# ilovin/lstm_ctc_ocr

Measured on NVIDIA H100. Metric: text-line images/sec (fwd+CTC loss), higher is better.
Workload: dtype bf16

## Files before the change

lstm_ctc_ocr_b200/csrc/backward.cu:

```cuda
#include <cmath>
#include <cstring>

#include "backward_kernels.cuh"
#include "conv1_wgrad_tc.cuh"
#include "conv_swap.cuh"
#include "gemm_launch.h"
#include "kernels.cuh"
#include "lstm_bwd.cuh"
#include "model_internal.h"

extern "C" int crnn_model_set_training(crnn_model* m, int flag) {
  if (!m) return crnn_fail(CRNN_INVALID_VALUE, "set_training: null model");
  if (flag && m->cfg.compute_dtype >= 2) return crnn_fail(CRNN_UNSUPPORTED, "set_training: the f32-class paths (compute_dtype 2, 3) are forward + CTC only");
  if (flag && !m->wblock_bwd) {
    const size_t nB[9] = {512 * 4608, 256 * 4608, 256 * 2304, 128 * 2304, 64 * 1152, 1024 * 1024, 512 * 64, 512 * 2048, 512 * 1024};
    size_t tot = 1024;
    for (size_t v : nB) tot += align_up(v * 2);
    CUDA_TRY(cudaMalloc(&m->wblock_bwd, tot));
    uint8_t* p = reinterpret_cast<uint8_t*>(m->wblock_bwd);
    __nv_bfloat16** dst[9] = {&m->Bd_c42, &m->Bd_c41, &m->Bd_c32, &m->Bd_c31, &m->Bd_c2, &m->Bd_c5, &m->Bld, &m->Bxb, &m->Bhb};
    for (int i = 0; i < 9; ++i) { *dst[i] = reinterpret_cast<__nv_bfloat16*>(p); p += align_up(nB[i] * 2); }
    m->grad_sumsq = reinterpret_cast<double*>(p);
    CRNN_TRY(make_tmap_2d(&m->tD_c42, m->Bd_c42, 512, 4608, 4608, 256));
    CRNN_TRY(make_tmap_2d(&m->tD_c41, m->Bd_c41, 256, 4608, 4608, 256));
// ... 102 lines not shown
    if (!attr) {
      CUDA_TRY(cudaFuncSetAttribute(lstm_bwd::lstm_bwd_kernel, cudaFuncAttributeMaxDynamicSharedMemorySize, lstm_bwd::SMEM_BYTES));
      CUDA_TRY(cudaFuncSetAttribute(lstm_bwd::lstm_bwd_ks_kernel, cudaFuncAttributeMaxDynamicSharedMemorySize, lstm_bwd::ks::SMEM_BYTES));
      attr = true;
    }
    cudaLaunchConfig_t cfg;
    memset(&cfg, 0, sizeof(cfg));
    cfg.gridDim = dim3(lstm_bwd::CS * 2 * lp.tiles_per_dir);
    cfg.blockDim = dim3(m->bptt_ks ? lstm_bwd::ks::NUM_THREADS : lstm_bwd::NUM_THREADS);
    cfg.dynamicSmemBytes = m->bptt_ks ? lstm_bwd::ks::SMEM_BYTES : lstm_bwd::SMEM_BYTES;
    cfg.stream = st;
    cudaLaunchAttribute at[1];
    at[0].id = cudaLaunchAttributeClusterDimension;
    at[0].val.clusterDim.x = lstm_bwd::CS; at[0].val.clusterDim.y = 1; at[0].val.clusterDim.z = 1;
    cfg.attrs = at; cfg.numAttrs = 1;
    if (m->bptt_ks) CUDA_TRY(cudaLaunchKernelEx(&cfg, lstm_bwd::lstm_bwd_ks_kernel, m->tD_h256, lp, pl.bptt_x));
    else CUDA_TRY(cudaLaunchKernelEx(&cfg, lstm_bwd::lstm_bwd_kernel, pl.tG_dzstate, m->tD_h, lp));
  }
  BMARK();
  {
    const std::string fw = "logits/bidirectional_rnn/fw/lstm_cell", bw = "logits/bidirectional_rnn/bw/lstm_cell";
    const long long dW = m->find(bw + "/weights")->offset - m->find(fw + "/weights")->offset;
    const long long db = m->find(bw + "/biases")->offset - m->find(fw + "/biases")->offset;
    CRNN_TRY(launch_colsum_bf16(pl.dz_all, R, 2048, G(fw + "/biases"), 32, db, st));
    {
      gemm_tn::Params p = tn_plain(512, 2048, R, G(fw + "/weights"), 1024);
      p.num_n_tiles = 8; p.lstm_cols = 1; p.dir_stride = dW;
      CRNN_TRY((launch_gemm_tn<256, gemm_tn::TN_PLAIN, 4>(pl.tT_a5, pl.tT_dz, p, sms, st)));
    }
    {
      gemm_tn::Params p = tn_plain(256, 1024, R, G(fw + "/weights"), 1024);
      p.num_n_tiles = 4; p.lstm_cols = 1; p.out_row_offset = 512; p.a_row_shift = -1;
// ... 216 lines not shown
```

lstm_ctc_ocr_b200/csrc/lstm.cuh:

```cuda
#pragma once
#include <cuda.h>

#include "common.cuh"
#include "wgmma.cuh"

namespace lstm {

constexpr int NUM_THREADS = 384;
constexpr int BLOCK_M = 128;

struct Params {
  const __nv_bfloat16* xproj;
  __nv_bfloat16* h_state;
  __nv_bfloat16* lstm_out;
  const int* seq_len;
  int Nimg, Npad, H, T, tiles_per_dir;
  __nv_bfloat16* gates;
  float* csave;
  int swap_ls;
  long long* trace;
};

#define LSTM_TRACE_WG(wg, ev)                                                                           \
  do {                                                                                                  \
    if (p.trace != nullptr && lane == 0 && s >= 8 && s < 12 && (blockIdx.x == 0 || blockIdx.x == 5))    \
      p.trace[((((blockIdx.x ? 1 : 0) * 2 + (wg)) * 4 + (s - 8)) * 16) + (ev)] = clock64();             \
  } while (0)
#define LSTM_TRACE(ev) LSTM_TRACE_WG(0, ev)

__device__ __forceinline__ uint32_t cluster_ctarank() {
  uint32_t r;
  asm volatile("mov.u32 %0, %%cluster_ctarank;" : "=r"(r));
  return r;
}
__device__ __forceinline__ void cluster_arrive_release() { asm volatile("barrier.cluster.arrive.release.aligned;" ::: "memory"); }
// ... 197 lines not shown
  static constexpr int HALF_ROWS = BLOCK_M / 2;
  static constexpr int HALF_A_BYTES = 32 * HALF_ROWS * 16;
  static constexpr int A_BYTES = 2 * HALF_A_BYTES;
  static constexpr int SLICE_BYTES = HALF_A_BYTES / CS;
  static constexpr int BAR_OFFSET = 2 * A_BYTES + B_BYTES;
  static constexpr int SMEM_BYTES = BAR_OFFSET + 128 + 1024;
};

__device__ __forceinline__ void bulk_copy_s2s_cluster(uint32_t dst_cluster_addr, const void* src_smem, uint32_t bytes,
                                                      uint32_t bar_cluster_addr) {
  asm volatile("cp.async.bulk.shared::cluster.shared::cta.mbarrier::complete_tx::bytes [%0], [%1], %2, [%3];" ::"r"(dst_cluster_addr),
               "r"(ptx::smem_u32(src_smem)), "r"(bytes), "r"(bar_cluster_addr)
               : "memory");
}

template <int CS, int MODE, int EW>
__global__ void __launch_bounds__(McThreads<EW>::ALL, 1)
lstm_mc_kernel(const __grid_constant__ CUtensorMap tmW, const Params p) {
  static_assert(CS == 8, "8 CTAs x 32 units");
  using C = CfgMc<CS>;
  constexpr int UPC = C::UPC, NCOLS = C::NCOLS;
  static_assert(EW == 8, "epilogue warps = the two MMA warpgroups");
  static_assert(NCOLS == 128, "fragment column group j = gate j/4, units 8(j%4) ..: one m64n128 product per half and step");
  constexpr bool DS = (MODE == 1), MS = (MODE == 2), GX = (MODE == 3), LOCAL = DS || MS;
  constexpr uint32_t FILL_TX = LOCAL ? (CS - 1) * C::SLICE_BYTES : C::HALF_A_BYTES;

  extern __shared__ uint8_t smem_raw[];
  uint8_t* smem = smem_raw + ((1024u - (ptx::smem_u32(smem_raw) & 1023u)) & 1023u);
  uint8_t* smem_a = smem;
  uint8_t* smem_b = smem + 2 * C::A_BYTES;
  uint64_t* a_full = reinterpret_cast<uint64_t*>(smem + C::BAR_OFFSET);
  uint64_t* b_full = a_full + 4;
  uint64_t* part_ready = b_full + 1;

  const int warp_idx = threadIdx.x >> 5, lane = threadIdx.x & 31;
  const int rank = (int)cluster_ctarank();
  const int unit = blockIdx.x / CS;
  const int dir = unit / p.tiles_per_dir;
  const int tile = unit - dir * p.tiles_per_dir;

  if (warp_idx == 0 && lane == 0) {
    ptx::prefetch_tmap(&tmW);
    for (int i = 0; i < 4; ++i) {
      ptx::mbar_init(&part_ready[i], CS);
      ptx::mbar_init(&a_full[i], GX ? 128 : LOCAL ? 2 : 1);
    }
    ptx::mbar_init(b_full, 1);
    ptx::fence_barrier_init();
    for (int hf = 0; hf < 2; ++hf) {
      if (!GX && p.T > 1) ptx::mbar_arrive_expect_tx(&a_full[2 * hf + 1], FILL_TX);
      if (!GX && p.T > 2) ptx::mbar_arrive_expect_tx(&a_full[2 * hf + 0], FILL_TX);
    }
    ptx::mbar_arrive_expect_tx(b_full, C::B_BYTES);
    for (int kb = 0; kb < 4; ++kb)
      ptx::tma_load_2d(&tmW, b_full, smem_b + kb * NCOLS * 128, kb * 64, dir * 1024 + rank * NCOLS);
  }
  __syncthreads();
  cluster_arrive_release();
  cluster_wait_acquire();

  if (warp_idx < 4) {
    ptx::setmaxnreg_dec<40>();
  } else {
    ptx::setmaxnreg_inc<232>();
    const int wgi = (warp_idx >> 2) - 1;
    const int w = warp_idx & 3, q4 = lane & 3;
    const int rr0 = 16 * w + (lane >> 2);
    int n[2], len[2];
    bool okn[2];
#pragma unroll
    for (int rh = 0; rh < 2; ++rh) {
      n[rh] = tile * BLOCK_M + wgi * C::HALF_ROWS + rr0 + 8 * rh;
      okn[rh] = n[rh] < p.Nimg;
      len[rh] = okn[rh] ? min(max(__ldg(p.seq_len + n[rh]), 0), p.T) : 0;
    }
    float cst[2][4][2];
#pragma unroll
    for (int rh = 0; rh < 2; ++rh)
#pragma unroll
      for (int k = 0; k < 4; ++k) { cst[rh][k][0] = 0.f; cst[rh][k][1] = 0.f; }
    uint64_t* my_full = a_full + 2 * wgi;
    uint64_t* my_ready = part_ready + 2 * wgi;
    ptx::mbar_wait(b_full, 0);
    const uint32_t word_off = rr0 * 16 + q4 * 4;
    uint8_t* hx_half = reinterpret_cast<uint8_t*>(p.h_state) + (size_t)(unit * 2 + wgi) * C::HALF_A_BYTES;
    const size_t hx_buf_stride = (size_t)2 * p.tiles_per_dir * C::A_BYTES;

    for (int s = 0; s < p.T; ++s) {
      bool active[2];
      int t[2];
      uint32_t xw[2][4][4];
#pragma unroll
      for (int rh = 0; rh < 2; ++rh) {
        active[rh] = s < len[rh];
        t[rh] = active[rh] ? (dir ? (len[rh] - 1 - s) : s) : s;
        if (active[rh]) {
          const uint32_t* src = reinterpret_cast<const uint32_t*>(p.xproj + ((size_t)n[rh] * p.H + s) * 2048 + dir * 1024 + rank * NCOLS + 2 * q4);
#pragma unroll
          for (int g = 0; g < 4; ++g)
#pragma unroll
            for (int k = 0; k < 4; ++k) xw[rh][g][k] = __ldg(src + (g * UPC + 8 * k) / 2);
// ... 79 lines not shown
                ptx::mbar_arrive(&my_full[nb]);
              } else {
                const uint32_t dst_peer = ptx::mapa(ptx::smem_u32(my_slice), (uint32_t)lane);
                const uint32_t bar = ptx::mapa(ptx::smem_u32(&my_full[nb]), (uint32_t)lane);
                bulk_copy_s2s_cluster(dst_peer, my_slice, C::SLICE_BYTES, bar);
              }
            }
          } else if (MS) {
            if (lane == 0) {
              ptx::bulk_store_1d(hx_slice, my_slice, C::SLICE_BYTES);
              ptx::bulk_commit();
              asm volatile("cp.async.bulk.wait_group 0;" ::: "memory");
              ptx::bulk_load_1d_mc(my_slice, hx_slice, C::SLICE_BYTES, &my_full[nb], (uint16_t)(((1u << CS) - 1) & ~(1u << rank)));
              ptx::mbar_arrive(&my_full[nb]);
            }
          } else if (GX) {
            if (lane < CS) ptx::mbar_arrive_cluster(ptx::mapa(ptx::smem_u32(&my_ready[nb]), (uint32_t)lane));
          } else if (lane == 0) {
            ptx::bulk_load_1d_mc(my_slice, hx_slice, C::SLICE_BYTES, &my_full[nb], (uint16_t)((1u << CS) - 1));
          }
          __syncwarp();
          LSTM_TRACE_WG(wgi, 9);
        }
        if (GX) {
          ptx::mbar_wait_cluster(&my_ready[nb], (uint32_t)(s >> 1) & 1u);
          const uint8_t* g = hx_half + (size_t)nb * hx_buf_stride;
          uint8_t* a = smem_a + nb * C::A_BYTES + wgi * C::HALF_A_BYTES;
          const int et = threadIdx.x & 127;
          uint4 v[C::HALF_A_BYTES / 16 / 128];
#pragma unroll
// ... 20 lines not shown
          for (int g = 0; g < 4; ++g)
#pragma unroll
            for (int k = 0; k < 4; ++k)
              *reinterpret_cast<uint32_t*>(gs + g * LSTM_GATE_STRIDE + k * LSTM_GCHUNK_STRIDE) =
                  ptx::pack_bf16x2(d[16 * g + 4 * k + 2 * rh], d[16 * g + 4 * k + 2 * rh + 1]);
#pragma unroll
          for (int k = 0; k < 4; ++k)
            *reinterpret_cast<float2*>(cs + (2 * k + (q4 >> 1)) * LSTM_CCHUNK_STRIDE) = make_float2(cst[rh][k][0], cst[rh][k][1]);
        }
      }
      if (w == 0) LSTM_TRACE_WG(wgi, 10);
    }
  }

  __syncthreads();
  cluster_arrive_release();
  cluster_wait_acquire();
}

}
```

lstm_ctc_ocr_b200/csrc/lstm_bwd.cuh:

```cuda
#pragma once
#include <cuda.h>

#include "common.cuh"
#include "lstm.cuh"
#include "wgmma.cuh"

namespace lstm_bwd {

constexpr int NUM_THREADS = 256;
constexpr int BLOCK_M = 128;
constexpr int CS = 8;
constexpr int UPC = 32;
constexpr int STAGES = 6;
constexpr int B_BYTES = 16 * UPC * 128;
constexpr int A_STAGE = BLOCK_M * 128;
constexpr int ACC_OFFSET = B_BYTES + STAGES * A_STAGE;
constexpr int BAR_OFFSET = ACC_OFFSET + BLOCK_M * UPC * 4;
constexpr int SMEM_BYTES = BAR_OFFSET + 256 + 1024;

struct Params {
  const __nv_bfloat16* gates;
  const float* csave;
  const __nv_bfloat16* d_out;
  __nv_bfloat16* dz_state;
  __nv_bfloat16* dz_all;
  const int* seq_len;
  int Nimg, Npad, H, T, tiles_per_dir;
};

__device__ __forceinline__ uint4 pack8(const float* v) {
  return make_uint4(ptx::pack_bf16x2(v[0], v[1]), ptx::pack_bf16x2(v[2], v[3]), ptx::pack_bf16x2(v[4], v[5]),
                    ptx::pack_bf16x2(v[6], v[7]));
}
__device__ __forceinline__ void unpack8(const uint4 q, float* v) {
  v[0] = ptx::bf16_lo(q.x); v[1] = ptx::bf16_hi(q.x); v[2] = ptx::bf16_lo(q.y); v[3] = ptx::bf16_hi(q.y);
  v[4] = ptx::bf16_lo(q.z); v[5] = ptx::bf16_hi(q.z); v[6] = ptx::bf16_lo(q.w); v[7] = ptx::bf16_hi(q.w);
}

__global__ void __launch_bounds__(NUM_THREADS, 1)
lstm_bwd_kernel(const __grid_constant__ CUtensorMap tmDz, const __grid_constant__ CUtensorMap tmW, const Params p) {
  extern __shared__ uint8_t smem_raw[];
  uint8_t* smem = reinterpret_cast<uint8_t*>((reinterpret_cast<uintptr_t>(smem_raw) + 1023) & ~uintptr_t(1023));
// ... 183 lines not shown
  extern __shared__ uint8_t smem_raw[];
  uint8_t* smem = smem_raw + ((1024u - (ptx::smem_u32(smem_raw) & 1023u)) & 1023u);
  uint8_t* smem_b = smem;
  uint8_t* smem_a = smem + ks::B_BYTES;
  float* acc_tile = reinterpret_cast<float*>(smem + ks::ACC_OFFSET);
  uint64_t* b_full = reinterpret_cast<uint64_t*>(smem + ks::BAR_OFFSET);
  uint64_t* a_ready = b_full + 1;
  uint64_t* part_ready = a_ready + 1;

  const int warp_idx = threadIdx.x >> 5, lane = threadIdx.x & 31;
  const int rank = (int)lstm::cluster_ctarank();
  const int unit = blockIdx.x / CS;
  const int dir = unit / p.tiles_per_dir;
  const int tile = unit - dir * p.tiles_per_dir;
  const int num_units = 2 * p.tiles_per_dir;

  if (warp_idx == 0 && lane == 0) {
    ptx::prefetch_tmap(&tmW);
    ptx::mbar_init(b_full, 1);
    ptx::mbar_init(a_ready, ks::EPI_THREADS);
    ptx::mbar_init(&part_ready[0], CS);
    ptx::mbar_init(&part_ready[1], CS);
    ptx::fence_barrier_init();
    ptx::mbar_arrive_expect_tx(b_full, ks::B_BYTES);
    for (int kb = 0; kb < 2; ++kb) ptx::tma_load_2d(&tmW, b_full, smem_b + kb * 256 * 128, rank * 128 + kb * 64, dir * 256);
  }
  __syncthreads();
  lstm::cluster_arrive_release();
  lstm::cluster_wait_acquire();

// ... 140 lines not shown
        ptx::mbar_arrive(a_ready);
      }
      if (okn) {
        __nv_bfloat16* za = p.dz_all + ((size_t)n * p.H + t) * 2048 + dir * 1024 + rank * 128 + u0;
        ptx::st_global_v8(za + 0 * 32, zi0.x, zi0.y, zi0.z, zi0.w, zi1.x, zi1.y, zi1.z, zi1.w);
        ptx::st_global_v8(za + 1 * 32, zj0.x, zj0.y, zj0.z, zj0.w, zj1.x, zj1.y, zj1.z, zj1.w);
        ptx::st_global_v8(za + 2 * 32, zf0.x, zf0.y, zf0.z, zf0.w, zf1.x, zf1.y, zf1.z, zf1.w);
        ptx::st_global_v8(za + 3 * 32, zo0.x, zo0.y, zo0.z, zo0.w, zo1.x, zo1.y, zo1.z, zo1.w);
      }
    }
  }

  __syncthreads();
  lstm::cluster_arrive_release();
  lstm::cluster_wait_acquire();
}

}
```

lstm_ctc_ocr_b200/csrc/model.cu:

```cuda
#include <cstdarg>
#include <cstring>
#include <string>
#include <vector>

#include <cstdlib>
#include <condition_variable>
#include <mutex>
#include <thread>

#include "gemm_launch.h"
#include "lstm.cuh"
#include "conv_swap.cuh"
#include "conv1_tc.cuh"
#include "kernels.cuh"
#include "model_internal.h"

static thread_local char g_err[1024] = "";
int crnn_fail(int status, const char* fmt, ...) {
  va_list ap;
  va_start(ap, fmt);
  vsnprintf(g_err, sizeof(g_err), fmt, ap);
  va_end(ap);
  return status;
}
// ... 147 lines not shown
  if (prop.major != 9) {
    delete m;
    return crnn_fail(CRNN_UNSUPPORTED, "model_create: needs sm_90 (found sm_%d%d)", prop.major, prop.minor);
  }
  m->num_sms = prop.multiProcessorCount;
  if (const char* e = getenv("CRNN_BPTT")) m->bptt_ks = std::string(e) != "ring";
  if (const char* e = getenv("CRNN_CONV1")) m->conv1_tc = std::string(e) != "simt";
  if (const char* e = getenv("CRNN_BN_FUSE")) m->bn_red_fused = std::string(e) != "0";
  if (const char* e = getenv("CRNN_RELU_FUSE")) m->relu_mask_fused = std::string(e) != "0";
  if (const char* e = getenv("CRNN_CONV1_WGRAD")) m->conv1_wgrad_tc = std::string(e) != "simt";
  if (const char* e = getenv("CRNN_CONV2_DGRAD")) m->conv2_dgrad_swap = std::string(e) != "old";
  if (const char* e = getenv("CRNN_CONV2_WGRAD")) m->conv2_wgrad_swap = std::string(e) != "old";
  if (const char* e = getenv("CRNN_CONV2")) m->conv2_swap = std::string(e) != "pos";
  if (const char* e = getenv("CRNN_LSTM_IMPL")) {
    m->lstm_upc = (std::string(e) == "step") ? 64 : 32;
    m->lstm_mc = std::string(e) == "ds" ? 2 : std::string(e) == "mc" ? 1 : std::string(e) == "gx" ? 4 : (std::string(e) == "persistent" || std::string(e) == "step") ? 0 : 3;
  }

  const size_t nB[9] = {128 * 576, 256 * 1152, 256 * 2304, 512 * 2304, 512 * 4608, 512 * 2048, 2048 * 512, 2048 * 256, 64 * 512};
  size_t tot = 0;
  for (size_t v : nB) tot += (v * 2 + 1023) / 1024 * 1024;
  tot += 2048 * 4 + 1024;
  if (cudaMalloc(&m->wblock, tot) != cudaSuccess) { delete m; return crnn_fail(CRNN_CUDA_ERROR, "model_create: cudaMalloc"); }
  uint8_t* p = reinterpret_cast<uint8_t*>(m->wblock);
  __nv_bfloat16** dst[9] = {&m->Bc2, &m->Bc31, &m->Bc32, &m->Bc41, &m->Bc42, &m->Bc5, &m->Bx, &m->Bh, &m->Bl};
  for (int i = 0; i < 9; ++i) { *dst[i] = reinterpret_cast<__nv_bfloat16*>(p); p += (nB[i] * 2 + 1023) / 1024 * 1024; }
  m->xbias = reinterpret_cast<float*>(p); p += 2048 * 4;
  m->sumsq = reinterpret_cast<double*>(p);
  int st = CRNN_OK;
  if (st == CRNN_OK) st = make_tmap_2d(&m->tB_c2, m->Bc2, 128, 576, 576, 128);
  if (st == CRNN_OK) st = make_tmap_2d(&m->tB_c31, m->Bc31, 256, 1152, 1152, 256);
// ... 4 lines not shown
  if (st == CRNN_OK) st = make_tmap_2d(&m->tB_x, m->Bx, 2048, 512, 512, 256);
  if (st == CRNN_OK) st = make_tmap_2d(&m->tB_h, m->Bh, 2048, 256, 256, 256);
  if (st == CRNN_OK) st = make_tmap_2d(&m->tB_h128, m->Bh, 2048, 256, 256, 128);
  if (st == CRNN_OK) st = make_tmap_2d(&m->tB_l, m->Bl, 64, 512, 512, 64);
  if (st != CRNN_OK) { cudaFree(m->wblock); delete m; return st; }
  *out = m;
  return CRNN_OK;
}

extern "C" int crnn_model_destroy(crnn_model* m) {
  if (!m) return CRNN_OK;
  x3_destroy(m);
  if (m->wblock) cudaFree(m->wblock);
  if (m->wblock_bwd) cudaFree(m->wblock_bwd);
  if (m->d_peers) cudaFree(m->d_peers);
  for (auto e : m->prof_events) cudaEventDestroy(e);
  for (auto e : m->prof_events_bwd) cudaEventDestroy(e);
  for (auto e : m->chunk_events) cudaEventDestroy(e);
  delete m;
  return CRNN_OK;
}
extern "C" int crnn_num_tensors(const crnn_model* m) { return m ? (int)m->tensors.size() : 0; }
extern "C" int64_t crnn_param_count(const crnn_model* m) { return m ? m->total : 0; }
extern "C" int crnn_param_info(const crnn_model* m, int index, const char** tf_name, int64_t* offset, int64_t shape[4],
                               int* ndim) {
  if (!m || index < 0 || index >= (int)m->tensors.size()) return crnn_fail(CRNN_INVALID_VALUE, "param_info: bad index");
  const TensorInfo& t = m->tensors[index];
  if (tf_name) *tf_name = t.name.c_str();
  if (offset) *offset = t.offset;
  if (shape) for (int k = 0; k < 4; ++k) shape[k] = t.shape[k];
// ... 27 lines not shown
    CRNN_TRY(launch_transpose_cast(w, 512, 1024, 1024, m->Bx + (size_t)d * 1024 * 512, 512, m->lstm_upc, st));
    CRNN_TRY(launch_transpose_cast(w + 512 * 1024, 256, 1024, 1024, m->Bh + (size_t)d * 1024 * 256, 256, m->lstm_upc, st));
  }
  CRNN_TRY(launch_lstm_bias_prep(m->P(std::string(dirs[0]) + "/biases"), m->P(std::string(dirs[1]) + "/biases"), m->xbias, m->lstm_upc, st));
  CRNN_TRY(launch_transpose_cast(m->P("logits/weights"), 512, 64, 64, m->Bl, 512, 0, st));
  SumsqSegs segs;
  segs.n = 0;
  for (auto& c : kConvs) {
    const TensorInfo* t = m->find(std::string(c.name) + "/weights");
    segs.off[segs.n] = t->offset; segs.cnt[segs.n] = t->count; segs.n++;
  }
  const TensorInfo* t = m->find("logits/weights");
  segs.off[segs.n] = t->offset; segs.cnt[segs.n] = t->count; segs.n++;
  CRNN_TRY(launch_sumsq(m->params, segs, m->sumsq, st));
  m->dirty = false;
  return CRNN_OK;
}

size_t align_up(size_t v, size_t a) { return (v + a - 1) / a * a; }

size_t layout_plan(Plan& pl, int N, int W, uint8_t* base, bool train) {
  pl.N = N; pl.W = W; pl.H1 = W / 2; pl.H2 = W / 4; pl.T = W / 4 - 1;
  pl.Npad = (N + 127) / 128 * 128;
  size_t off = 0;
  auto take = [&](size_t bytes) { uint8_t* p = base ? base + off : nullptr; off += align_up(bytes); return p; };
  const size_t n = N, h1 = pl.H1, h2 = pl.H2;
  pl.a1 = (__nv_bfloat16*)take(n * h1 * 16 * 64 * 2);
  pl.a2 = (__nv_bfloat16*)take(n * h2 * 8 * 128 * 2);
  pl.a3 = (__nv_bfloat16*)take(n * h2 * 8 * 256 * 2);
  pl.a3p = (__nv_bfloat16*)take(n * h2 * 4 * 256 * 2);
  pl.a4a_pre = (__nv_bfloat16*)take(n * h2 * 4 * 512 * 2);
  pl.a4a = (__nv_bfloat16*)take(n * h2 * 4 * 512 * 2);
  pl.a4b_pre = (__nv_bfloat16*)take(n * h2 * 4 * 512 * 2);
  pl.a4b = (__nv_bfloat16*)take(n * h2 * 2 * 512 * 2);
  pl.a5 = (__nv_bfloat16*)take(n * h2 * 512 * 2);
  pl.xproj = (__nv_bfloat16*)take(n * h2 * 2048 * 2);
  pl.lstm_out = (__nv_bfloat16*)take(n * h2 * 512 * 2);
  pl.h_state = (__nv_bfloat16*)take((size_t)2 * 2 * pl.Npad * 256 * 2);
  pl.c_state = (float*)take((size_t)2 * pl.Npad * 256 * 4);
  pl.stats = (double*)take(2 * 2 * 512 * 8);
  pl.bn = (float*)take(2 * 4 * 512 * 4);
  pl.train = train;
  if (train) {
    const size_t T = pl.T;
    pl.am1 = (uint8_t*)take(n * h1 * 16 * 64);
    pl.am2 = (uint8_t*)take(n * h2 * 8 * 128);
    pl.am3 = (uint8_t*)take(n * h2 * 4 * 256);
    pl.gates = (__nv_bfloat16*)take((size_t)2 * pl.Npad * T * 1024 * 2);
    pl.csave = (float*)take((size_t)2 * pl.Npad * T * 256 * 4);
    pl.dl_rows = (__nv_bfloat16*)take(n * h2 * 64 * 2);
    pl.d_lstm_out = (__nv_bfloat16*)take(n * h2 * 512 * 2);
    pl.dz_all = (__nv_bfloat16*)take(n * h2 * 2048 * 2);
    pl.dz_state = (__nv_bfloat16*)take((size_t)2 * 2 * pl.Npad * 1024 * 2);
// ... 315 lines not shown
    else CRNN_TRY((launch_gemm<256, gemm::A_PLAIN, gemm::EPI_BIAS_BF16, 4>(pl.tA_x, m->tB_x, p, sms, st, &pl.tO_x)));
  }
  STAGE_MARK();
  if (m->lstm_upc == 32) {
    constexpr int CS = 8;
    lstm::Params lp;
    lp.xproj = pl.xproj; lp.h_state = pl.h_state; lp.lstm_out = pl.lstm_out; lp.seq_len = time_step_len;
    lp.Nimg = N; lp.Npad = pl.Npad; lp.H = H2; lp.T = T; lp.tiles_per_dir = pl.Npad / 128;
    lp.gates = pl.train ? pl.gates : nullptr; lp.csave = pl.train ? pl.csave : nullptr;
    static long long* d_trace = nullptr;
    const bool want_trace = getenv("CRNN_LSTM_TRACE") != nullptr;
    if (want_trace && d_trace == nullptr) CUDA_TRY(cudaMalloc(&d_trace, 2 * 2 * 4 * 16 * sizeof(long long)));
    if (want_trace) CUDA_TRY(cudaMemsetAsync(d_trace, 0, 2 * 2 * 4 * 16 * sizeof(long long), st));
    lp.trace = want_trace ? d_trace : nullptr;
    lp.swap_ls = getenv("CRNN_LSTM_SWAPLS") != nullptr;
    auto kern = lstm::lstm_persistent_kernel<CS>;
    auto kern_mc = lstm::lstm_mc_kernel<CS, 0, 8>;
    auto kern_ds = lstm::lstm_mc_kernel<CS, 1, 8>;
    auto kern_ms = lstm::lstm_mc_kernel<CS, 2, 8>;
    auto kern_gx = lstm::lstm_mc_kernel<CS, 3, 8>;
    static bool attr = false;
    if (!attr) {
      CUDA_TRY(cudaFuncSetAttribute(kern, cudaFuncAttributeMaxDynamicSharedMemorySize, lstm::Cfg<CS>::SMEM_BYTES));
      CUDA_TRY(cudaFuncSetAttribute(kern_mc, cudaFuncAttributeMaxDynamicSharedMemorySize, lstm::CfgMc<CS>::SMEM_BYTES));
      CUDA_TRY(cudaFuncSetAttribute(kern_ds, cudaFuncAttributeMaxDynamicSharedMemorySize, lstm::CfgMc<CS>::SMEM_BYTES));
      CUDA_TRY(cudaFuncSetAttribute(kern_ms, cudaFuncAttributeMaxDynamicSharedMemorySize, lstm::CfgMc<CS>::SMEM_BYTES));
      CUDA_TRY(cudaFuncSetAttribute(kern_gx, cudaFuncAttributeMaxDynamicSharedMemorySize, lstm::CfgMc<CS>::SMEM_BYTES));
      attr = true;
    }
    cudaLaunchConfig_t cfg;
    memset(&cfg, 0, sizeof(cfg));
    cfg.gridDim = dim3(CS * 2 * lp.tiles_per_dir);
    cfg.blockDim = dim3(m->lstm_mc ? lstm::McThreads<8>::ALL : lstm::NUM_THREADS);
    cfg.dynamicSmemBytes = m->lstm_mc ? lstm::CfgMc<CS>::SMEM_BYTES : lstm::Cfg<CS>::SMEM_BYTES;
    cfg.stream = st;
    cudaLaunchAttribute at[1];
    at[0].id = cudaLaunchAttributeClusterDimension;
    at[0].val.clusterDim.x = CS; at[0].val.clusterDim.y = 1; at[0].val.clusterDim.z = 1;
    cfg.attrs = at; cfg.numAttrs = 1;
    if (m->lstm_mc == 4) CUDA_TRY(cudaLaunchKernelEx(&cfg, kern_gx, m->tB_h128, lp));
    else if (m->lstm_mc == 3) CUDA_TRY(cudaLaunchKernelEx(&cfg, kern_ms, m->tB_h128, lp));
    else if (m->lstm_mc == 2) CUDA_TRY(cudaLaunchKernelEx(&cfg, kern_ds, m->tB_h128, lp));
    else if (m->lstm_mc == 1) CUDA_TRY(cudaLaunchKernelEx(&cfg, kern_mc, m->tB_h128, lp));
    else CUDA_TRY(cudaLaunchKernelEx(&cfg, kern, pl.tA_hall, m->tB_h128, lp));
    if (want_trace) {
      long long h[2 * 2 * 4 * 16];
      CUDA_TRY(cudaStreamSynchronize(st));
      CUDA_TRY(cudaMemcpy(h, d_trace, sizeof(h), cudaMemcpyDeviceToHost));
      for (int c = 0; c < 2; ++c) {
        long long t0 = 0;
        for (int i = c * 128; i < (c + 1) * 128; ++i)
          if (h[i] && (!t0 || h[i] < t0)) t0 = h[i];
        for (int wg = 0; wg < 2; ++wg)
          for (int s = 0; s < 4; ++s) {
            const long long* r = h + ((c * 2 + wg) * 4 + s) * 16;
            bool any = false;
            for (int e = 0; e < 16; ++e) any = any || r[e];
            if (!any) continue;
            fprintf(stderr, "lstm_trace cta%d wg%d step%d:", c ? 5 : 0, wg, 8 + s);
// ... 196 lines not shown
```

lstm_ctc_ocr_b200/csrc/model_internal.h:

```cpp
#pragma once
#include <string>
#include <vector>

#include <cuda.h>

#include "common.cuh"
#include "gemm.cuh"

int make_tmap_2d(CUtensorMap* m, const void* base, uint64_t rows, uint64_t cols, uint64_t row_stride, uint32_t box_rows);
int make_tmap_nhwc(CUtensorMap* m, const void* base, int N, int H, int Wd, int C, int bh);
int make_tmap_2d_f32(CUtensorMap* m, const void* base, uint64_t rows, uint64_t cols, uint64_t row_stride, uint32_t box_rows);
int make_tmap_nhwc_f32(CUtensorMap* m, const void* base, int N, int H, int Wd, int C, int bh);
size_t align_up(size_t v, size_t a = 1024);
int make_tmap_2d_box(CUtensorMap* m, const void* base, uint64_t rows, uint64_t cols, uint64_t row_stride, uint32_t box_cols,
                     uint32_t box_rows);

struct TensorInfo {
  std::string name;
  int ndim;
  int64_t shape[4];
  int64_t offset;
  int64_t count;
};

// ... 6 lines not shown
static const char* kStageNames[] = {"conv1_pool1", "conv2_pool2", "conv3_1", "conv3_2_pool", "conv4_1_gemm", "bn4_1_apply",
                                    "conv4_2_gemm", "bn4_2_apply_pool3", "conv5", "lstm_xproj", "lstm_recurrence", "logits"};
static const int kNumStages = 12;
static const char* kBwdStageNames[] = {"zero+logits_bwd", "lstm_bptt", "lstm_wgrad+dx", "conv5_bwd", "bn4_2_bwd", "conv4_2_wgrad",
                                       "conv4_2_dgrad", "bn4_1_bwd", "conv4_1_wgrad", "conv4_1_dgrad", "conv3_2_bwd_elem", "conv3_2_wgrad",
                                       "conv3_2_dgrad", "conv3_1_bwd_elem", "conv3_1_wgrad", "conv3_1_dgrad", "conv2_bwd_elem", "conv2_wgrad",
                                       "conv2_dgrad", "conv1_wgrad"};
static const int kNumBwdStages = 20;

static const int kMaxChunks = 16;

struct Plan {
  int N = 0, W = 0, H1 = 0, H2 = 0, T = 0, Npad = 0;
  void* ws = nullptr;
  __nv_bfloat16 *a1, *a2, *a3, *a3p, *a4a_pre, *a4a, *a4b_pre, *a4b, *a5, *xproj, *lstm_out, *h_state;
  float* c_state;
  double* stats;
  float* bn;
  CUtensorMap tA_c2s;
  CUtensorMap tA_c2, tA_c31, tA_c32, tA_c41, tA_c42, tA_c5, tA_x, tA_h[2], tA_l, tA_hall;
  CUtensorMap tO_c1, tO_c2s, tO_c32, tO_c41, tO_c42, tO_x;
  int mg2 = 0, mg3 = 0, mg4 = 0, wm2 = 0, wm3 = 0, wm4 = 0;
  CUtensorMap tW_a1, tW_a2, tW_a3, tW_a3p, tW_a4a, tW_p4b, tW_p4a, tW_p32, tW_p31, tW_p2;
  bool train = false;
  uint8_t *am1, *am2, *am3;
  __nv_bfloat16* gates;
  float* csave;
  __nv_bfloat16 *dl_rows, *d_lstm_out, *dz_all, *dz_state, *d_a5, *d_a4b, *d_pre4b, *d_pre4a, *d_a3p, *d_pre32, *d_pre31, *d_a2,
      *d_pre2, *d_a1;
  uint8_t* bptt_x;
// ... 21 lines not shown
  bool dirty_bwd = true;
  void* wblock_bwd = nullptr;
  __nv_bfloat16 *Bd_c42 = nullptr, *Bd_c41, *Bd_c32, *Bd_c31, *Bd_c2, *Bd_c5, *Bld, *Bxb, *Bhb;
  CUtensorMap tD_c42, tD_c41, tD_c32, tD_c31, tD_c2, tD_c5, tD_l, tD_x, tD_h;
  CUtensorMap tDs_c2;
  CUtensorMap tD_h256;
  bool bptt_ks = true;
  double* grad_sumsq = nullptr;
  bool conv1_tc = true;
  bool bn_red_fused = true;
  bool relu_mask_fused = true;
  bool conv1_wgrad_tc = true;
  bool conv2_dgrad_swap = true;
  bool conv2_wgrad_swap = true;
  bool conv2_swap = true;
  int lstm_mc = 3;
  int lstm_upc = 32;
  Plan plan;
  void* x3 = nullptr;
  int dp_rank = 0, dp_world = 1;
  crnn_allreduce_fn xchg_cb = nullptr;
  void* xchg_user = nullptr;
  void** d_peers = nullptr;
  int* d_peer_err = nullptr;
  unsigned long long peer_epoch = 0;
  int bwd_sm_reserve = 0;
  crnn_grad_ready_fn grad_cb = nullptr;
  void* grad_user = nullptr;
  std::vector<cudaEvent_t> chunk_events;
  std::vector<cudaEvent_t> prof_events;
  int prof_slots = 0, prof_used = 0;
// ... 8 lines not shown
  float* P(const std::string& n) const { return params + find(n)->offset; }
};

size_t x3_workspace_size(int N, int W);
int x3_forward(crnn_model* m, const float* data, const int* time_step_len, int N, int W, float* logits_out, void* workspace,
               size_t workspace_bytes, cudaStream_t st);
int x3_debug_tap(crnn_model* m, const char* name, float* dst, size_t dst_elems, void* workspace, cudaStream_t st);
int x3_debug_tap_raw(crnn_model* m, const char* name, void* dst, size_t dst_bytes, void* workspace, cudaStream_t st);
void x3_destroy(crnn_model* m);
void x3_params_changed(crnn_model* m);

int dp_allreduce_1024(crnn_model* m, const double* in, double* out, cudaStream_t st);
int dp_allreduce_bn_finalize(crnn_model* m, double* stats, double count_global, const float* gamma, const float* beta, float eps,
                             float* bn , cudaStream_t st);

size_t layout_plan(Plan& pl, int N, int W, uint8_t* base, bool train);
int prepare_weights(crnn_model* m, cudaStream_t st);
int ensure_plan(crnn_model* m, int N, int W, void* ws, cudaStream_t st);

static inline gemm::Params conv_params(int N, int H, int Wd, int Cin, int Cout, int block_n, const float* bias, void* out,
                                       int merged = 0) {
  gemm::Params p;
  memset(&p, 0, sizeof(p));
  p.bh = 32 / Wd;
  p.Wd = Wd; p.H = H; p.Nimg = N;
  p.sb_per_img = (H + p.bh - 1) / p.bh;
  p.num_m_tiles = (N * p.sb_per_img + 3) / 4;
  p.num_n_tiles = Cout / block_n;
  p.cin_blocks = Cin / 64;
  p.num_k_blocks = 9 * p.cin_blocks;
// ... 9 lines not shown
```

lstm_ctc_ocr_b200/csrc/ptx.cuh:

```cuda
#pragma once
#include <cuda_runtime.h>
#include <cuda_bf16.h>
#include <stdint.h>

namespace ptx {

__device__ __forceinline__ uint32_t smem_u32(const void* p) {
  return static_cast<uint32_t>(__cvta_generic_to_shared(p));
}
__device__ __forceinline__ uint32_t lane_id() { return threadIdx.x & 31; }

__device__ __forceinline__ bool elect_one() {
  uint32_t pred = 0;
  asm volatile(
      "{\n\t.reg .pred p;\n\t"
      "elect.sync _|p, 0xffffffff;\n\t"
      "selp.u32 %0, 1, 0, p;\n\t}\n"
      : "=r"(pred));
  return pred != 0;
}

__device__ __forceinline__ void mbar_init(uint64_t* bar, uint32_t count) {
  asm volatile("mbarrier.init.shared::cta.b64 [%0], %1;" ::"r"(smem_u32(bar)), "r"(count));
}
// ... 163 lines not shown
__device__ __forceinline__ void mbar_wait_cluster(uint64_t* bar, uint32_t parity) {
  uint32_t ok;
  do {
    asm volatile(
        "{\n\t.reg .pred p;\n\t"
        "mbarrier.try_wait.parity.acquire.cluster.shared::cta.b64 p, [%1], %2;\n\t"
        "selp.u32 %0, 1, 0, p;\n\t}\n"
        : "=r"(ok)
        : "r"(smem_u32(bar)), "r"(parity)
        : "memory");
  } while (!ok);
}
__device__ __forceinline__ void mbar_arrive_cluster(uint32_t cluster_addr) {
  asm volatile("mbarrier.arrive.release.cluster.shared::cluster.b64 _, [%0];" ::"r"(cluster_addr) : "memory");
}
__device__ __forceinline__ void tma_load_2d_mc(const void* tmap, uint64_t* bar, void* dst, int c0, int c1, uint16_t cta_mask) {
  asm volatile(
      "cp.async.bulk.tensor.2d.shared::cluster.global.tile.mbarrier::complete_tx::bytes.multicast::cluster [%0], [%1, {%3, %4}], [%2], %5;"
      ::"r"(smem_u32(dst)), "l"(reinterpret_cast<uint64_t>(tmap)), "r"(smem_u32(bar)), "r"(c0), "r"(c1), "h"(cta_mask)
      : "memory");
}
__device__ __forceinline__ uint32_t pack_bf16x2(float lo, float hi) {
  __nv_bfloat162 t = __floats2bfloat162_rn(lo, hi);
  return *reinterpret_cast<uint32_t*>(&t);
}
__device__ __forceinline__ uint32_t hmax2_bf16(uint32_t a, uint32_t b) {
  __nv_bfloat162 x = *reinterpret_cast<__nv_bfloat162*>(&a);
  __nv_bfloat162 y = *reinterpret_cast<__nv_bfloat162*>(&b);
  __nv_bfloat162 r = __hmax2(x, y);
  return *reinterpret_cast<uint32_t*>(&r);
// ... 44 lines not shown
```

Measured before the change: 140,900.

## Add global-memory flag exchange LSTM mode and auto-select it when clusters don't fit

```diff
diff --git a/lstm_ctc_ocr_b200/csrc/backward.cu b/lstm_ctc_ocr_b200/csrc/backward.cu
--- a/lstm_ctc_ocr_b200/csrc/backward.cu
+++ b/lstm_ctc_ocr_b200/csrc/backward.cu
@@ -140,8 +140,11 @@
     at[0].id = cudaLaunchAttributeClusterDimension;
     at[0].val.clusterDim.x = lstm_bwd::CS; at[0].val.clusterDim.y = 1; at[0].val.clusterDim.z = 1;
     cfg.attrs = at; cfg.numAttrs = 1;
+    lp.waves = m->bptt_ks ? lstm_waves_buffer((int)cfg.gridDim.x, st) : nullptr;
     if (m->bptt_ks) CUDA_TRY(cudaLaunchKernelEx(&cfg, lstm_bwd::lstm_bwd_ks_kernel, m->tD_h256, lp, pl.bptt_x));
     else CUDA_TRY(cudaLaunchKernelEx(&cfg, lstm_bwd::lstm_bwd_kernel, pl.tG_dzstate, m->tD_h, lp));
+    if (lp.waves != nullptr)
+      CRNN_TRY(lstm_waves_report("bptt", lp.waves, (int)cfg.gridDim.x, (const void*)lstm_bwd::lstm_bwd_ks_kernel, cfg, st));
   }
   BMARK();
   {
diff --git a/lstm_ctc_ocr_b200/csrc/lstm.cuh b/lstm_ctc_ocr_b200/csrc/lstm.cuh
--- a/lstm_ctc_ocr_b200/csrc/lstm.cuh
+++ b/lstm_ctc_ocr_b200/csrc/lstm.cuh
@@ -19,6 +19,10 @@
   float* csave;
   int swap_ls;
   long long* trace;
+  unsigned long long* waves;
+  int unit_base;
+  unsigned* h_flags;
+  int* err;
 };
 
 #define LSTM_TRACE_WG(wg, ev)                                                                           \
@@ -246,6 +250,8 @@
                : "memory");
 }
 
+constexpr long long GG_SPIN_LIMIT = 4000000000ll;
+
 template <int CS, int MODE, int EW>
 __global__ void __launch_bounds__(McThreads<EW>::ALL, 1)
 lstm_mc_kernel(const __grid_constant__ CUtensorMap tmW, const Params p) {
@@ -254,7 +260,8 @@
   constexpr int UPC = C::UPC, NCOLS = C::NCOLS;
   static_assert(EW == 8, "epilogue warps = the two MMA warpgroups");
   static_assert(NCOLS == 128, "fragment column group j = gate j/4, units 8(j%4) ..: one m64n128 product per half and step");
-  constexpr bool DS = (MODE == 1), MS = (MODE == 2), GX = (MODE == 3), LOCAL = DS || MS;
+  constexpr bool DS = (MODE == 1), MS = (MODE == 2), GX = (MODE == 3), GG = (MODE == 4);
+  constexpr bool LOCAL = DS || MS || GG;
   constexpr uint32_t FILL_TX = LOCAL ? (CS - 1) * C::SLICE_BYTES : C::HALF_A_BYTES;
 
   extern __shared__ uint8_t smem_raw[];
@@ -266,10 +273,11 @@
   uint64_t* part_ready = b_full + 1;
 
   const int warp_idx = threadIdx.x >> 5, lane = threadIdx.x & 31;
-  const int rank = (int)cluster_ctarank();
-  const int unit = blockIdx.x / CS;
+  const int rank = GG ? (int)(blockIdx.x % CS) : (int)cluster_ctarank();
+  const int unit = (GG ? p.unit_base : 0) + (int)(blockIdx.x / CS);
   const int dir = unit / p.tiles_per_dir;
   const int tile = unit - dir * p.tiles_per_dir;
+  if (p.waves != nullptr && threadIdx.x == 0) p.waves[2 * (unit * CS + rank)] = ptx::globaltimer();
 
   if (warp_idx == 0 && lane == 0) {
     ptx::prefetch_tmap(&tmW);
@@ -288,8 +296,10 @@
       ptx::tma_load_2d(&tmW, b_full, smem_b + kb * NCOLS * 128, kb * 64, dir * 1024 + rank * NCOLS);
   }
   __syncthreads();
-  cluster_arrive_release();
-  cluster_wait_acquire();
+  if (!GG) {
+    cluster_arrive_release();
+    cluster_wait_acquire();
+  }
 
   if (warp_idx < 4) {
     ptx::setmaxnreg_dec<40>();
@@ -317,6 +327,7 @@
     const uint32_t word_off = rr0 * 16 + q4 * 4;
     uint8_t* hx_half = reinterpret_cast<uint8_t*>(p.h_state) + (size_t)(unit * 2 + wgi) * C::HALF_A_BYTES;
     const size_t hx_buf_stride = (size_t)2 * p.tiles_per_dir * C::A_BYTES;
+    bool timed_out = false;
 
     for (int s = 0; s < p.T; ++s) {
       bool active[2];
@@ -426,6 +437,29 @@
               ptx::bulk_load_1d_mc(my_slice, hx_slice, C::SLICE_BYTES, &my_full[nb], (uint16_t)(((1u << CS) - 1) & ~(1u << rank)));
               ptx::mbar_arrive(&my_full[nb]);
             }
+          } else if (GG) {
+            if (lane == 0) {
+              ptx::bulk_store_1d(hx_slice, my_slice, C::SLICE_BYTES);
+              ptx::bulk_commit();
+              ptx::bulk_wait_all();
+              ptx::fence_proxy_async_global();
+              unsigned* flag = p.h_flags + (unit * 2 + wgi) * 2 + nb;
+              ptx::red_release_gpu_add(flag, 1u);
+              const unsigned want = (unsigned)CS * (unsigned)((s >> 1) + 1);
+              if (!timed_out) {
+                const long long t0 = clock64();
+                while (ptx::ld_acquire_gpu(flag) < want) {
+                  if (clock64() - t0 > GG_SPIN_LIMIT) { timed_out = true; atomicExch(p.err, 1); break; }
+                }
+              }
+              ptx::fence_proxy_async_global();
+              const uint8_t* src = hx_half + (size_t)nb * hx_buf_stride;
+              uint8_t* dst = smem_a + nb * C::A_BYTES + wgi * C::HALF_A_BYTES;
+              if (rank > 0) ptx::bulk_load_1d(dst, src, rank * C::SLICE_BYTES, &my_full[nb]);
+              if (rank < CS - 1)
+                ptx::bulk_load_1d(dst + (rank + 1) * C::SLICE_BYTES, src + (rank + 1) * C::SLICE_BYTES, (CS - 1 - rank) * C::SLICE_BYTES, &my_full[nb]);
+              ptx::mbar_arrive(&my_full[nb]);
+            }
           } else if (GX) {
             if (lane < CS) ptx::mbar_arrive_cluster(ptx::mapa(ptx::smem_u32(&my_ready[nb]), (uint32_t)lane));
           } else if (lane == 0) {
@@ -476,8 +510,11 @@
   }
 
   __syncthreads();
-  cluster_arrive_release();
-  cluster_wait_acquire();
+  if (!GG) {
+    cluster_arrive_release();
+    cluster_wait_acquire();
+  }
+  if (p.waves != nullptr && threadIdx.x == 0) p.waves[2 * (unit * CS + rank) + 1] = ptx::globaltimer();
 }
 
 }
diff --git a/lstm_ctc_ocr_b200/csrc/lstm_bwd.cuh b/lstm_ctc_ocr_b200/csrc/lstm_bwd.cuh
--- a/lstm_ctc_ocr_b200/csrc/lstm_bwd.cuh
+++ b/lstm_ctc_ocr_b200/csrc/lstm_bwd.cuh
@@ -26,6 +26,7 @@
   __nv_bfloat16* dz_all;
   const int* seq_len;
   int Nimg, Npad, H, T, tiles_per_dir;
+  unsigned long long* waves;
 };
 
 __device__ __forceinline__ uint4 pack8(const float* v) {
@@ -239,6 +240,7 @@
   const int dir = unit / p.tiles_per_dir;
   const int tile = unit - dir * p.tiles_per_dir;
   const int num_units = 2 * p.tiles_per_dir;
+  if (p.waves != nullptr && threadIdx.x == 0) p.waves[2 * blockIdx.x] = ptx::globaltimer();
 
   if (warp_idx == 0 && lane == 0) {
     ptx::prefetch_tmap(&tmW);
@@ -409,6 +411,7 @@
   __syncthreads();
   lstm::cluster_arrive_release();
   lstm::cluster_wait_acquire();
-}
-
-}
+  if (p.waves != nullptr && threadIdx.x == 0) p.waves[2 * blockIdx.x + 1] = ptx::globaltimer();
+}
+
+}
diff --git a/lstm_ctc_ocr_b200/csrc/model.cu b/lstm_ctc_ocr_b200/csrc/model.cu
--- a/lstm_ctc_ocr_b200/csrc/model.cu
+++ b/lstm_ctc_ocr_b200/csrc/model.cu
@@ -1,3 +1,4 @@
+#include <algorithm>
 #include <cstdarg>
 #include <cstring>
 #include <string>
@@ -185,7 +186,8 @@
   if (const char* e = getenv("CRNN_CONV2")) m->conv2_swap = std::string(e) != "pos";
   if (const char* e = getenv("CRNN_LSTM_IMPL")) {
     m->lstm_upc = (std::string(e) == "step") ? 64 : 32;
-    m->lstm_mc = std::string(e) == "ds" ? 2 : std::string(e) == "mc" ? 1 : std::string(e) == "gx" ? 4 : (std::string(e) == "persistent" || std::string(e) == "step") ? 0 : 3;
+    const std::string v(e);
+    m->lstm_mc = v == "ds" ? 2 : v == "mc" ? 1 : v == "gx" ? 4 : v == "ms" ? 3 : v == "gg" ? 5 : (v == "persistent" || v == "step") ? 0 : 6;
   }
 
   const size_t nB[9] = {128 * 576, 256 * 1152, 256 * 2304, 512 * 2304, 512 * 4608, 512 * 2048, 2048 * 512, 2048 * 256, 64 * 512};
@@ -220,6 +222,7 @@
   if (m->wblock) cudaFree(m->wblock);
   if (m->wblock_bwd) cudaFree(m->wblock_bwd);
   if (m->d_peers) cudaFree(m->d_peers);
+  if (m->lstm_err) cudaFreeHost(m->lstm_err);
   for (auto e : m->prof_events) cudaEventDestroy(e);
   for (auto e : m->prof_events_bwd) cudaEventDestroy(e);
   for (auto e : m->chunk_events) cudaEventDestroy(e);
@@ -277,6 +280,56 @@
   segs.off[segs.n] = t->offset; segs.cnt[segs.n] = t->count; segs.n++;
   CRNN_TRY(launch_sumsq(m->params, segs, m->sumsq, st));
   m->dirty = false;
+  return CRNN_OK;
+}
+
+unsigned long long* lstm_waves_buffer(int ctas, cudaStream_t st) {
+  static const bool on = getenv("CRNN_LSTM_WAVES") != nullptr;
+  static unsigned long long* buf = nullptr;
+  static int cap = 0;
+  if (!on) return nullptr;
+  if (ctas > cap) {
+    if (buf) cudaFree(buf);
+    buf = nullptr; cap = 0;
+    if (cudaMalloc(&buf, (size_t)ctas * 2 * sizeof(unsigned long long)) != cudaSuccess) return nullptr;
+    cap = ctas;
+  }
+  if (cudaMemsetAsync(buf, 0, (size_t)ctas * 2 * sizeof(unsigned long long), st) != cudaSuccess) return nullptr;
+  return buf;
+}
+
+int lstm_waves_report(const char* name, const unsigned long long* buf, int ctas, const void* func, const cudaLaunchConfig_t& cfg,
+                      cudaStream_t st) {
+  bool cluster = false;
+  for (unsigned i = 0; i < cfg.numAttrs; ++i) cluster = cluster || cfg.attrs[i].id == cudaLaunchAttributeClusterDimension;
+  int dev = 0, sms = 0, per_sm = 0, clusters = -1;
+  CUDA_TRY(cudaGetDevice(&dev));
+  CUDA_TRY(cudaDeviceGetAttribute(&sms, cudaDevAttrMultiProcessorCount, dev));
+  CUDA_TRY(cudaOccupancyMaxActiveBlocksPerMultiprocessor(&per_sm, func, (int)cfg.blockDim.x, cfg.dynamicSmemBytes));
+  if (cluster) CUDA_TRY(cudaOccupancyMaxActiveClusters(&clusters, func, &cfg));
+  std::vector<unsigned long long> h((size_t)ctas * 2);
+  CUDA_TRY(cudaStreamSynchronize(st));
+  CUDA_TRY(cudaMemcpy(h.data(), buf, h.size() * sizeof(unsigned long long), cudaMemcpyDeviceToHost));
+  const int units = ctas / 8;
+  std::vector<unsigned long long> us(units, ~0ull), ue(units, 0ull);
+  unsigned long long t0 = ~0ull;
+  for (int c = 0; c < ctas; ++c) {
+    us[c / 8] = std::min(us[c / 8], h[2 * c]);
+    ue[c / 8] = std::max(ue[c / 8], h[2 * c + 1]);
+    t0 = std::min(t0, h[2 * c]);
+  }
+  std::vector<unsigned long long> sorted(us);
+  std::sort(sorted.begin(), sorted.end());
+  int groups = 0;
+  unsigned long long first = 0;
+  for (int u = 0; u < units; ++u)
+    if (u == 0 || sorted[u] > first + 3000) { ++groups; first = sorted[u]; }
+  fprintf(stderr, "lstm_waves %s: %d CTAs = %d units of 8, block %u threads, %zu B smem; co-resident: %d CTA(s)/SM x %d SMs", name,
+          ctas, units, cfg.blockDim.x, cfg.dynamicSmemBytes, per_sm, sms);
+  if (cluster) fprintf(stderr, ", max active 8-CTA clusters %d", clusters);
+  fprintf(stderr, "; start groups %d\n", groups);
+  for (int u = 0; u < units; ++u)
+    fprintf(stderr, "lstm_waves %s unit %d: start %.2f us end %.2f us\n", name, u, (us[u] - t0) * 1e-3, (ue[u] - t0) * 1e-3);
   return CRNN_OK;
 }
 
@@ -300,6 +353,7 @@
   pl.xproj = (__nv_bfloat16*)take(n * h2 * 2048 * 2);
   pl.lstm_out = (__nv_bfloat16*)take(n * h2 * 512 * 2);
   pl.h_state = (__nv_bfloat16*)take((size_t)2 * 2 * pl.Npad * 256 * 2);
+  pl.lstm_flags = (unsigned*)take((size_t)(2 * pl.Npad / 128) * 2 * 2 * sizeof(unsigned));
   pl.c_state = (float*)take((size_t)2 * pl.Npad * 256 * 4);
   pl.stats = (double*)take(2 * 2 * 512 * 8);
   pl.bn = (float*)take(2 * 4 * 512 * 4);
@@ -645,11 +699,15 @@
     if (want_trace) CUDA_TRY(cudaMemsetAsync(d_trace, 0, 2 * 2 * 4 * 16 * sizeof(long long), st));
     lp.trace = want_trace ? d_trace : nullptr;
     lp.swap_ls = getenv("CRNN_LSTM_SWAPLS") != nullptr;
+    const int units = 2 * lp.tiles_per_dir;
+    lp.waves = lstm_waves_buffer(units * CS, st);
+    lp.unit_base = 0; lp.h_flags = pl.lstm_flags; lp.err = nullptr;
     auto kern = lstm::lstm_persistent_kernel<CS>;
     auto kern_mc = lstm::lstm_mc_kernel<CS, 0, 8>;
     auto kern_ds = lstm::lstm_mc_kernel<CS, 1, 8>;
     auto kern_ms = lstm::lstm_mc_kernel<CS, 2, 8>;
     auto kern_gx = lstm::lstm_mc_kernel<CS, 3, 8>;
+    auto kern_gg = lstm::lstm_mc_kernel<CS, 4, 8>;
     static bool attr = false;
     if (!attr) {
       CUDA_TRY(cudaFuncSetAttribute(kern, cudaFuncAttributeMaxDynamicSharedMemorySize, lstm::Cfg<CS>::SMEM_BYTES));
@@ -657,11 +715,12 @@
       CUDA_TRY(cudaFuncSetAttribute(kern_ds, cudaFuncAttributeMaxDynamicSharedMemorySize, lstm::CfgMc<CS>::SMEM_BYTES));
       CUDA_TRY(cudaFuncSetAttribute(kern_ms, cudaFuncAttributeMaxDynamicSharedMemorySize, lstm::CfgMc<CS>::SMEM_BYTES));
       CUDA_TRY(cudaFuncSetAttribute(kern_gx, cudaFuncAttributeMaxDynamicSharedMemorySize, lstm::CfgMc<CS>::SMEM_BYTES));
+      CUDA_TRY(cudaFuncSetAttribute(kern_gg, cudaFuncAttributeMaxDynamicSharedMemorySize, lstm::CfgMc<CS>::SMEM_BYTES));
       attr = true;
     }
     cudaLaunchConfig_t cfg;
     memset(&cfg, 0, sizeof(cfg));
-    cfg.gridDim = dim3(CS * 2 * lp.tiles_per_dir);
+    cfg.gridDim = dim3(CS * units);
     cfg.blockDim = dim3(m->lstm_mc ? lstm::McThreads<8>::ALL : lstm::NUM_THREADS);
     cfg.dynamicSmemBytes = m->lstm_mc ? lstm::CfgMc<CS>::SMEM_BYTES : lstm::Cfg<CS>::SMEM_BYTES;
     cfg.stream = st;
@@ -669,11 +728,41 @@
     at[0].id = cudaLaunchAttributeClusterDimension;
     at[0].val.clusterDim.x = CS; at[0].val.clusterDim.y = 1; at[0].val.clusterDim.z = 1;
     cfg.attrs = at; cfg.numAttrs = 1;
-    if (m->lstm_mc == 4) CUDA_TRY(cudaLaunchKernelEx(&cfg, kern_gx, m->tB_h128, lp));
-    else if (m->lstm_mc == 3) CUDA_TRY(cudaLaunchKernelEx(&cfg, kern_ms, m->tB_h128, lp));
-    else if (m->lstm_mc == 2) CUDA_TRY(cudaLaunchKernelEx(&cfg, kern_ds, m->tB_h128, lp));
-    else if (m->lstm_mc == 1) CUDA_TRY(cudaLaunchKernelEx(&cfg, kern_mc, m->tB_h128, lp));
+    const void* launched = nullptr;
+    int mode = m->lstm_mc;
+    if (mode == 6) {
+      if (m->lstm_ms_clusters < 0) CUDA_TRY(cudaOccupancyMaxActiveClusters(&m->lstm_ms_clusters, kern_ms, &cfg));
+      mode = units <= m->lstm_ms_clusters ? 3 : 5;
+    }
+    if (mode == 5) {
+      if (m->lstm_err == nullptr) {
+        CUDA_TRY(cudaHostAlloc(&m->lstm_err, sizeof(int), cudaHostAllocMapped));
+        *m->lstm_err = 0;
+      }
+      if (*(volatile int*)m->lstm_err)
+        return crnn_fail(CRNN_CUDA_ERROR, "lstm recurrence: a CTA waited more than ~2 s for a peer's h slice in an earlier launch");
+      if (m->lstm_gg_units == 0) {
+        int per_sm = 0;
+        CUDA_TRY(cudaOccupancyMaxActiveBlocksPerMultiprocessor(&per_sm, kern_gg, lstm::McThreads<8>::ALL, lstm::CfgMc<CS>::SMEM_BYTES));
+        m->lstm_gg_units = per_sm * m->num_sms / CS;
+        if (m->lstm_gg_units < 1) return crnn_fail(CRNN_UNSUPPORTED, "lstm recurrence: 8 CTAs of lstm_mc_kernel do not fit on this GPU at once");
+      }
+      lp.err = m->lstm_err;
+      CUDA_TRY(cudaMemsetAsync(pl.lstm_flags, 0, (size_t)units * 2 * 2 * sizeof(unsigned), st));
+      at[0].id = cudaLaunchAttributeCooperative;
+      at[0].val.cooperative = 1;
+      for (int u0 = 0; u0 < units; u0 += m->lstm_gg_units) {
+        lp.unit_base = u0;
+        cfg.gridDim = dim3(CS * std::min(m->lstm_gg_units, units - u0));
+        CUDA_TRY(cudaLaunchKernelEx(&cfg, kern_gg, m->tB_h128, lp));
+      }
+      launched = (const void*)kern_gg;
+    } else if (mode == 4) { CUDA_TRY(cudaLaunchKernelEx(&cfg, kern_gx, m->tB_h128, lp)); launched = (const void*)kern_gx; }
+    else if (mode == 3) { CUDA_TRY(cudaLaunchKernelEx(&cfg, kern_ms, m->tB_h128, lp)); launched = (const void*)kern_ms; }
+    else if (mode == 2) { CUDA_TRY(cudaLaunchKernelEx(&cfg, kern_ds, m->tB_h128, lp)); launched = (const void*)kern_ds; }
+    else if (mode == 1) { CUDA_TRY(cudaLaunchKernelEx(&cfg, kern_mc, m->tB_h128, lp)); launched = (const void*)kern_mc; }
     else CUDA_TRY(cudaLaunchKernelEx(&cfg, kern, pl.tA_hall, m->tB_h128, lp));
+    if (lp.waves != nullptr && launched != nullptr) CRNN_TRY(lstm_waves_report("forward", lp.waves, units * CS, launched, cfg, st));
     if (want_trace) {
       long long h[2 * 2 * 4 * 16];
       CUDA_TRY(cudaStreamSynchronize(st));
diff --git a/lstm_ctc_ocr_b200/csrc/model_internal.h b/lstm_ctc_ocr_b200/csrc/model_internal.h
--- a/lstm_ctc_ocr_b200/csrc/model_internal.h
+++ b/lstm_ctc_ocr_b200/csrc/model_internal.h
@@ -44,6 +44,7 @@
   int N = 0, W = 0, H1 = 0, H2 = 0, T = 0, Npad = 0;
   void* ws = nullptr;
   __nv_bfloat16 *a1, *a2, *a3, *a3p, *a4a_pre, *a4a, *a4b_pre, *a4b, *a5, *xproj, *lstm_out, *h_state;
+  unsigned* lstm_flags;
   float* c_state;
   double* stats;
   float* bn;
@@ -95,7 +96,10 @@
   bool conv2_dgrad_swap = true;
   bool conv2_wgrad_swap = true;
   bool conv2_swap = true;
-  int lstm_mc = 3;
+  int lstm_mc = 6;
+  int lstm_ms_clusters = -1;
+  int lstm_gg_units = 0;
+  int* lstm_err = nullptr;
   int lstm_upc = 32;
   Plan plan;
   void* x3 = nullptr;
@@ -134,6 +138,10 @@
 int dp_allreduce_bn_finalize(crnn_model* m, double* stats, double count_global, const float* gamma, const float* beta, float eps,
                              float* bn , cudaStream_t st);
 
+unsigned long long* lstm_waves_buffer(int ctas, cudaStream_t st);
+int lstm_waves_report(const char* name, const unsigned long long* buf, int ctas, const void* func, const cudaLaunchConfig_t& cfg,
+                      cudaStream_t st);
+
 size_t layout_plan(Plan& pl, int N, int W, uint8_t* base, bool train);
 int prepare_weights(crnn_model* m, cudaStream_t st);
 int ensure_plan(crnn_model* m, int N, int W, void* ws, cudaStream_t st);
diff --git a/lstm_ctc_ocr_b200/csrc/ptx.cuh b/lstm_ctc_ocr_b200/csrc/ptx.cuh
--- a/lstm_ctc_ocr_b200/csrc/ptx.cuh
+++ b/lstm_ctc_ocr_b200/csrc/ptx.cuh
@@ -201,6 +201,20 @@
 __device__ __forceinline__ void mbar_arrive_cluster(uint32_t cluster_addr) {
   asm volatile("mbarrier.arrive.release.cluster.shared::cluster.b64 _, [%0];" ::"r"(cluster_addr) : "memory");
 }
+__device__ __forceinline__ void red_release_gpu_add(unsigned* p, unsigned v) {
+  asm volatile("red.release.gpu.global.add.u32 [%0], %1;" ::"l"(p), "r"(v) : "memory");
+}
+__device__ __forceinline__ unsigned ld_acquire_gpu(const unsigned* p) {
+  unsigned v;
+  asm volatile("ld.acquire.gpu.global.u32 %0, [%1];" : "=r"(v) : "l"(p) : "memory");
+  return v;
+}
+__device__ __forceinline__ void fence_proxy_async_global() { asm volatile("fence.proxy.async.global;" ::: "memory"); }
+__device__ __forceinline__ unsigned long long globaltimer() {
+  unsigned long long t;
+  asm volatile("mov.u64 %0, %%globaltimer;" : "=l"(t));
+  return t;
+}
 __device__ __forceinline__ void tma_load_2d_mc(const void* tmap, uint64_t* bar, void* dst, int c0, int c1, uint16_t cta_mask) {
   asm volatile(
       "cp.async.bulk.tensor.2d.shared::cluster.global.tile.mbarrier::complete_tx::bytes.multicast::cluster [%0], [%1, {%3, %4}], [%2], %5;"
```

New measurement: 144,100 (median of 6 runs). +2.3%, better.
